# FengDushuo/BBBP-Multi-Modal-Deep-Ensemble-Framework

Hardware: AMD Instinct MI355X
Metric: molecules/sec fwd+bwd (3-branch ensemble, B=512) (higher is better)
Workload: dtype f32; 1 GPU; MixedInputModel F=167 (MACCS) + 3x128x128 image, 6-layer encoder + 2-stage CNN + fusion + BN head; forward + MSE + backward + fused AdamW, train mode (dropout 0.1); global_batch=512, per_gpu_batch=512, parallelism=dp1, input=device-resident

## Files before the change

### bbbp-multi-modal-deep-ensemble-framework_amd/csrc/head.hip

```cpp
#include "common.h"
#include "bbbp_hip.h"
#include "head_sync.h"

namespace {

constexpr int ROWS = 16;
constexpr int NTH = 512;
constexpr int NW = NTH / 64;
constexpr int COMB = 256, FHID = 128, NHEADS = 4, H1 = 256, H2 = 128, H3 = 64;
constexpr int LD = COMB + 4;
typedef float f32x4g __attribute__((ext_vector_type(4), aligned(4)));
static_assert(NTH >= H1, "one thread per BatchNorm column");

struct HeadParams {
    const float* comb;
    const float* fw1[NHEADS]; const float* fb1[NHEADS]; const float* fw2[NHEADS]; const float* fb2[NHEADS];
    const float* w0; const float* b0;
    const float* gamma; const float* beta; float* running_mean; float* running_var;
    const float* w3; const float* b3;
    const float* w5; const float* b5;
    const float* w7; const float* b7;
    float* hid; float* attn; float* fused; float* h; float* hb; float* bn_mean; float* bn_rstd; float* h2; float* h3; float* out;
    float* partial;
    int B, training;
    float eps, momentum;
    int concat;
    int world, rank;
};

template <int NCH>
__device__ __forceinline__ void load_b(f32x4 (&bf)[NCH], const float* Wrow ) {
#pragma unroll
    for (int c = 0; c < NCH; ++c) { f32x4g v = *reinterpret_cast<const f32x4g*>(Wrow + 16 * c); bf[c] = f32x4{v[0], v[1], v[2], v[3]}; }
}
template <int NCH>
__device__ __forceinline__ f32x4 mma_tile(const f32x4 (&af)[NCH], const f32x4 (&bf)[NCH]) {
    f32x4 acc0 = {0.f, 0.f, 0.f, 0.f}, acc1 = {0.f, 0.f, 0.f, 0.f};
#pragma unroll
    for (int c = 0; c < NCH; ++c)
#pragma unroll
        for (int j = 0; j < 4; j += 2) {
            acc0 = __builtin_amdgcn_mfma_f32_16x16x4f32(af[c][j], bf[c][j], acc0, 0, 0, 0);
            acc1 = __builtin_amdgcn_mfma_f32_16x16x4f32(af[c][j + 1], bf[c][j + 1], acc1, 0, 0, 0);
        }
    return acc0 + acc1;
}

template <int NCH>
__device__ __forceinline__ void load_a(f32x4 (&af)[NCH], const float* s, int ld, int lane) {
    const int i = lane & 15, kq = lane >> 4;
#pragma unroll
    for (int c = 0; c < NCH; ++c) af[c] = *reinterpret_cast<const f32x4*>(s + i * ld + 16 * c + 4 * kq);
}

__device__ __forceinline__ float sum16(float v) {
    v += __shfl_xor(v, 1); v += __shfl_xor(v, 2); v += __shfl_xor(v, 4); v += __shfl_xor(v, 8);
    return v;
}

__global__ __launch_bounds__(NTH) void head_a_kernel(HeadParams p) {
    __shared__ __attribute__((aligned(16))) float sC[ROWS * LD];
    __shared__ float sLogit[NW][NHEADS][ROWS];
    __shared__ float sP[ROWS][NHEADS];
    const int t = threadIdx.x, lane = t & 63, wave = t >> 6;
    const int q = lane & 15, kq = lane >> 4;
    const int r0 = blockIdx.x * ROWS, nrows = min(ROWS, p.B - r0);
    for (int idx = t; idx < ROWS * (COMB / 4); idx += NTH) {
        const int r = idx / (COMB / 4), c4 = idx % (COMB / 4);
        f32x4 v = {0.f, 0.f, 0.f, 0.f};
        if (r < nrows) v = *reinterpret_cast<const f32x4*>(p.comb + (long)(r0 + r) * COMB + c4 * 4);
        *reinterpret_cast<f32x4*>(sC + r * LD + c4 * 4) = v;
    }
    __syncthreads();
    f32x4 af[COMB / 16];
    load_a<COMB / 16>(af, sC, LD, lane);
    float lg[NHEADS][4];
    f32x4 bf[2][COMB / 16];
    const int n = wave * 16 + q;
    if (p.concat) {
        load_b<COMB / 16>(bf[0], p.w0 + (long)n * COMB + 4 * kq);
    } else {
    load_b<COMB / 16>(bf[0], p.fw1[0] + (long)n * COMB + 4 * kq);
#pragma unroll
    for (int h = 0; h < NHEADS; ++h) {
        if (h + 1 < NHEADS) load_b<COMB / 16>(bf[(h + 1) & 1], p.fw1[h + 1] + (long)n * COMB + 4 * kq);
        else load_b<COMB / 16>(bf[(h + 1) & 1], p.w0 + (long)n * COMB + 4 * kq);
        f32x4 acc = mma_tile<COMB / 16>(af, bf[h & 1]);
        const float b = p.fb1[h][n], w2 = p.fw2[h][n];
#pragma unroll
        for (int r = 0; r < 4; ++r) {
            const int row = 4 * kq + r;
            const float v = tanhf(acc[r] + b);
            if (row < nrows) p.hid[((long)h * p.B + r0 + row) * FHID + n] = v;
            lg[h][r] = sum16(v * w2);
        }
    }
    if (q == 0) {
#pragma unroll
        for (int h = 0; h < NHEADS; ++h)
#pragma unroll
            for (int r = 0; r < 4; ++r) sLogit[wave][h][4 * kq + r] = lg[h][r];
    }
    __syncthreads();
    if (t < ROWS) {
        float a[NHEADS], m = -INFINITY;
#pragma unroll
        for (int h = 0; h < NHEADS; ++h) {
            float z = 0.f;
#pragma unroll
            for (int w = 0; w < NW; ++w) z += sLogit[w][h][t];
            a[h] = z + p.fb2[h][0];
            m = fmaxf(m, a[h]);
        }
        float den = 0.f;
#pragma unroll
        for (int h = 0; h < NHEADS; ++h) { a[h] = __expf(a[h] - m); den += a[h]; }
#pragma unroll
        for (int h = 0; h < NHEADS; ++h) {
            a[h] /= den;
            sP[t][h] = a[h];
            if (t < nrows) p.attn[(long)(r0 + t) * NHEADS + h] = a[h];
        }
    }
    __syncthreads();
    for (int idx = t; idx < ROWS * COMB; idx += NTH) {
        const int r = idx / COMB, c = idx % COMB;
        const float x = sC[r * LD + c];
        float s = 0.f;
#pragma unroll
        for (int h = 0; h < NHEADS; ++h) s += sP[r][h] * x;
        sC[r * LD + c] = s;
        if (r < nrows) p.fused[(long)(r0 + r) * COMB + c] = s;
    }
    __syncthreads();
    load_a<COMB / 16>(af, sC, LD, lane);
    }
#pragma unroll
    for (int tt = 0; tt < 2; ++tt) {
        const int n0 = (wave + NW * tt) * 16 + q;
        if (tt == 0) load_b<COMB / 16>(bf[1], p.w0 + (long)((wave + NW) * 16 + q) * COMB + 4 * kq);
        f32x4 acc = mma_tile<COMB / 16>(af, bf[tt & 1]);
        const float b = p.b0[n0];
        float v[4], s = 0.f;
#pragma unroll
        for (int r = 0; r < 4; ++r) {
            const int row = 4 * kq + r;
            v[r] = fmaxf(acc[r] + b, 0.f);
            if (row < nrows) { p.h[(long)(r0 + row) * H1 + n0] = v[r]; s += v[r]; }
        }
        s += __shfl_xor(s, 16); s += __shfl_xor(s, 32);
        const float mean = s / nrows;
        float m2 = 0.f;
#pragma unroll
        for (int r = 0; r < 4; ++r) if (4 * kq + r < nrows) { const float d = v[r] - mean; m2 += d * d; }
        m2 += __shfl_xor(m2, 16); m2 += __shfl_xor(m2, 32);
        if (kq == 0) {
            const long slot = (long)p.rank * gridDim.x + blockIdx.x;
            p.partial[(slot * 2 + 0) * H1 + n0] = mean;
            p.partial[(slot * 2 + 1) * H1 + n0] = m2;
        }
    }
}

__global__ __launch_bounds__(NTH) void head_b_kernel(HeadParams p) {
    __shared__ __attribute__((aligned(16))) float sA[ROWS * LD];
    __shared__ __attribute__((aligned(16))) float sB[ROWS * (H2 + 4)];
    __shared__ __attribute__((aligned(16))) float sD[ROWS * (H3 + 4)];
    __shared__ float sMean[H1], sRstd[H1];
    const int t = threadIdx.x, lane = t & 63, wave = t >> 6;
    const int q = lane & 15, kq = lane >> 4;
    const int r0 = blockIdx.x * ROWS, nrows = min(ROWS, p.B - r0);
    const int nblocks = (p.B + ROWS - 1) / ROWS;
    f32x4 bf3[H1 / 16];
    load_b<H1 / 16>(bf3, p.w3 + (long)(wave * 16 + q) * H1 + 4 * kq);
    if (t < H1) {
        const int c = t;
        float mean, rstd;
        if (p.training) {
            float na = 0.f, ma = 0.f, m2a = 0.f;
            for (int b = 0; b < nblocks * p.world; ++b) {
                const float nb = (float)min(ROWS, p.B - (b % nblocks) * ROWS);
                const float mb = p.partial[((long)b * 2 + 0) * H1 + c], m2b = p.partial[((long)b * 2 + 1) * H1 + c];
                const float d = mb - ma, n = na + nb;
                ma += d * (nb / n);
                m2a += m2b + d * d * (na * nb / n);
                na = n;
            }
            const float nall = (float)p.B * (float)p.world;
            const float var = m2a / nall;
            mean = ma; rstd = rsqrtf(var + p.eps);
            if (blockIdx.x == 0) {
                p.running_mean[c] = (1.f - p.momentum) * p.running_mean[c] + p.momentum * mean;
                p.running_var[c] = (1.f - p.momentum) * p.running_var[c] + p.momentum * var * (nall / (nall - 1.f));
            }
        } else {
            mean = p.running_mean[c]; rstd = rsqrtf(p.running_var[c] + p.eps);
        }
        sMean[c] = mean; sRstd[c] = rstd;
        if (blockIdx.x == 0) { p.bn_mean[c] = mean; p.bn_rstd[c] = rstd; }
    }
    __syncthreads();
    for (int idx = t; idx < ROWS * H1; idx += NTH) {
        const int r = idx / H1, c = idx % H1;
        float v = 0.f;
        if (r < nrows) {
            v = (p.h[(long)(r0 + r) * H1 + c] - sMean[c]) * sRstd[c] * p.gamma[c] + p.beta[c];
            p.hb[(long)(r0 + r) * H1 + c] = v;
        }
        sA[r * LD + c] = v;
    }
    __syncthreads();
    {
        f32x4 af[H1 / 16];
        load_a<H1 / 16>(af, sA, LD, lane);
        const int n = wave * 16 + q;
        f32x4 acc = mma_tile<H1 / 16>(af, bf3);
        const float b = p.b3[n];
#pragma unroll
        for (int r = 0; r < 4; ++r) {
            const int row = 4 * kq + r;
            const float v = fmaxf(acc[r] + b, 0.f);
            sB[row * (H2 + 4) + n] = v;
            if (row < nrows) p.h2[(long)(r0 + row) * H2 + n] = v;
        }
    }
    __syncthreads();
    if (wave < H3 / 16) {
        f32x4 af[H2 / 16], bf[H2 / 16];
        const int n = wave * 16 + q;
        load_b<H2 / 16>(bf, p.w5 + (long)n * H2 + 4 * kq);
        load_a<H2 / 16>(af, sB, H2 + 4, lane);
        f32x4 acc = mma_tile<H2 / 16>(af, bf);
        const float b = p.b5[n];
#pragma unroll
        for (int r = 0; r < 4; ++r) {
            const int row = 4 * kq + r;
            const float v = fmaxf(acc[r] + b, 0.f);
            sD[row * (H3 + 4) + n] = v;
            if (row < nrows) p.h3[(long)(r0 + row) * H3 + n] = v;
        }
    }
    __syncthreads();
    if (wave == 0) {
        const int row = lane >> 2, part = lane & 3;
        float s = 0.f;
#pragma unroll
        for (int k = 0; k < H3 / 4; ++k) s += sD[row * (H3 + 4) + part * (H3 / 4) + k] * p.w7[part * (H3 / 4) + k];
        s += __shfl_xor(s, 1); s += __shfl_xor(s, 2);
        if (part == 0 && row < nrows) p.out[r0 + row] = s + p.b7[0];
    }
}

struct HeadBwdParams {
    const float* dout;
    const float* comb; const float* hid; const float* attn; const float* h; const float* h2; const float* h3;
    const float* bn_mean; const float* bn_rstd; const float* gamma;
    const float* fw1[NHEADS]; const float* fw2[NHEADS];
    const float* w0; const float* w3; const float* w5; const float* w7;
    float* dh3; float* dh2; float* dhb; float* dh; float* dlogit; float* dpre; float* dcomb;
    float* dgamma; float* dbeta;
    float* partial;
    int B, training;
    int world, rank;
};

typedef float f32x2g __attribute__((ext_vector_type(2), aligned(4)));

template <int K, int T>
__device__ __forceinline__ void mma_kmajor(f32x4 (&acc)[T], const float* sA, int lda, const float* W, int ldw, int colbase, int lane) {
    const int q = lane & 15, kq = lane >> 4;
    const float* wcol = W + colbase + T * q;
#pragma unroll 4
    for (int c = 0; c < K / 16; ++c) {
        const f32x4 a = *reinterpret_cast<const f32x4*>(sA + q * lda + 16 * c + 4 * kq);
#pragma unroll
        for (int j = 0; j < 4; ++j) {
            const float* wr = wcol + (long)(16 * c + 4 * kq + j) * ldw;
            if constexpr (T == 2) {
                const f32x2g b = *reinterpret_cast<const f32x2g*>(wr);
                acc[0] = __builtin_amdgcn_mfma_f32_16x16x4f32(a[j], b[0], acc[0], 0, 0, 0);
                acc[1] = __builtin_amdgcn_mfma_f32_16x16x4f32(a[j], b[1], acc[1], 0, 0, 0);
            } else {
                acc[0] = __builtin_amdgcn_mfma_f32_16x16x4f32(a[j], wr[0], acc[0], 0, 0, 0);
            }
        }
    }
}

constexpr int LD2 = H2 + 4, LD3 = H3 + 4, LDP = FHID + 4;

__global__ __launch_bounds__(NTH) void head_bwd_a_kernel(HeadBwdParams p) {
    __shared__ __attribute__((aligned(16))) float sD3[ROWS * LD3];
    __shared__ __attribute__((aligned(16))) float sD2[ROWS * LD2];
    __shared__ float sPa[4][H1], sPb[4][H1];
    const int t = threadIdx.x, lane = t & 63, wave = t >> 6;
    const int q = lane & 15, kq = lane >> 4;
    const int r0 = blockIdx.x * ROWS, nrows = min(ROWS, p.B - r0);
    for (int idx = t; idx < ROWS * H3; idx += NTH) {
        const int r = idx / H3, c = idx % H3;
        float v = 0.f;
        if (r < nrows) {
            v = p.h3[(long)(r0 + r) * H3 + c] > 0.f ? p.dout[r0 + r] * p.w7[c] : 0.f;
            p.dh3[(long)(r0 + r) * H3 + c] = v;
        }
        sD3[r * LD3 + c] = v;
    }
    __syncthreads();
    {
        f32x4 acc[1] = {{0.f, 0.f, 0.f, 0.f}};
        mma_kmajor<H3, 1>(acc, sD3, LD3, p.w5, H2, wave * 16, lane);
        const int n = wave * 16 + q;
#pragma unroll
        for (int r = 0; r < 4; ++r) {
            const int row = 4 * kq + r;
            float v = 0.f;
            if (row < nrows) {
                v = p.h2[(long)(r0 + row) * H2 + n] > 0.f ? acc[0][r] : 0.f;
                p.dh2[(long)(r0 + row) * H2 + n] = v;
            }
            sD2[row * LD2 + n] = v;
        }
    }
    __syncthreads();
    {
        f32x4 acc[2] = {{0.f, 0.f, 0.f, 0.f}, {0.f, 0.f, 0.f, 0.f}};
        mma_kmajor<H2, 2>(acc, sD2, LD2, p.w3, H1, wave * 32, lane);
#pragma unroll
        for (int u = 0; u < 2; ++u) {
            const int n = wave * 32 + 2 * q + u;
            const float mu = p.bn_mean[n], rs = p.bn_rstd[n];
            float pa = 0.f, pb = 0.f;
#pragma unroll
            for (int r = 0; r < 4; ++r) {
                const int row = 4 * kq + r;
                if (row < nrows) {
                    const float g = acc[u][r];
                    p.dhb[(long)(r0 + row) * H1 + n] = g;
                    pa += g * (p.h[(long)(r0 + row) * H1 + n] - mu) * rs;
                    pb += g;
                }
            }
            sPa[kq][n] = pa; sPb[kq][n] = pb;
        }
    }
    __syncthreads();
    if (t < H1) {
        const long slot = (long)p.rank * gridDim.x + blockIdx.x;
        p.partial[(slot * 2 + 0) * H1 + t] = ((sPa[0][t] + sPa[1][t]) + sPa[2][t]) + sPa[3][t];
        p.partial[(slot * 2 + 1) * H1 + t] = ((sPb[0][t] + sPb[1][t]) + sPb[2][t]) + sPb[3][t];
    }
}

__global__ __launch_bounds__(NTH) void head_bwd_c_kernel(HeadBwdParams p) {
    __shared__ __attribute__((aligned(16))) float sX[ROWS * LD];
    __shared__ __attribute__((aligned(16))) float sP[NHEADS * ROWS * LDP];
    __shared__ float sSa[H1], sSb[H1];
    const int t = threadIdx.x, lane = t & 63, wave = t >> 6;
    const int q = lane & 15, kq = lane >> 4;
    const int r0 = blockIdx.x * ROWS, nrows = min(ROWS, p.B - r0);
    const int nblocks = (p.B + ROWS - 1) / ROWS;
    if (t < H1) {
        float sa = 0.f, sb = 0.f, la = 0.f, lb = 0.f;
        for (int b = 0; b < nblocks * p.world; ++b) {
            const float va = p.partial[((long)b * 2 + 0) * H1 + t], vb = p.partial[((long)b * 2 + 1) * H1 + t];
            sa += va; sb += vb;
            if (b / nblocks == p.rank) { la += va; lb += vb; }
        }
        sSa[t] = sa; sSb[t] = sb;
        if (blockIdx.x == 0) { p.dgamma[t] = la; p.dbeta[t] = lb; }
    }
    __syncthreads();
    for (int idx = t; idx < ROWS * H1; idx += NTH) {
        const int r = idx / H1, c = idx % H1;
        float v = 0.f;
        if (r < nrows) {
            const float d = p.dhb[(long)(r0 + r) * H1 + c], xv = p.h[(long)(r0 + r) * H1 + c];
            const float g = p.gamma[c], mu = p.bn_mean[c], rs = p.bn_rstd[c];
            const float nall = (float)p.B * (float)p.world;
            v = p.training ? g * rs * (d - sSb[c] / nall - (xv - mu) * rs * (sSa[c] / nall)) : d * g * rs;
            v = xv > 0.f ? v : 0.f;
            p.dh[(long)(r0 + r) * H1 + c] = v;
        }
        sX[r * LD + c] = v;
    }
    __syncthreads();
    f32x4 df[2] = {{0.f, 0.f, 0.f, 0.f}, {0.f, 0.f, 0.f, 0.f}};
    mma_kmajor<H1, 2>(df, sX, LD, p.w0, COMB, wave * 32, lane);
    __syncthreads();
#pragma unroll
    for (int u = 0; u < 2; ++u)
#pragma unroll
        for (int r = 0; r < 4; ++r) sX[(4 * kq + r) * LD + wave * 32 + 2 * q + u] = df[u][r];
    __syncthreads();
#pragma unroll
    for (int rr = 0; rr < 2; ++rr) {
        const int r = wave * 2 + rr;
        const bool live = r < nrows;
        float a[NHEADS], asum = 0.f;
#pragma unroll
        for (int hh = 0; hh < NHEADS; ++hh) { a[hh] = live ? p.attn[(long)(r0 + r) * NHEADS + hh] : 0.f; asum += a[hh]; }
        float tt = 0.f;
#pragma unroll
        for (int c = lane; c < COMB; c += 64) {
            const float g = sX[r * LD + c];
            tt += live ? g * p.comb[(long)(r0 + r) * COMB + c] : 0.f;
            sX[r * LD + c] = g * asum;
        }
#pragma unroll
        for (int o = 32; o > 0; o >>= 1) tt += __shfl_xor(tt, o);
#pragma unroll
        for (int hh = 0; hh < NHEADS; ++hh) {
            const float dl = a[hh] * (tt - tt * asum);
            if (lane == 0 && live) p.dlogit[(long)hh * p.B + r0 + r] = dl;
#pragma unroll
            for (int c = lane; c < FHID; c += 64) {
                float v = 0.f;
                if (live) {
                    const float y = p.hid[((long)hh * p.B + r0 + r) * FHID + c];
                    v = dl * p.fw2[hh][c] * (1.f - y * y);
                    p.dpre[((long)hh * p.B + r0 + r) * FHID + c] = v;
                }
                sP[(hh * ROWS + r) * LDP + c] = v;
            }
        }
    }
    __syncthreads();
    f32x4 acc[2] = {{0.f, 0.f, 0.f, 0.f}, {0.f, 0.f, 0.f, 0.f}};
#pragma unroll
    for (int hh = 0; hh < NHEADS; ++hh) mma_kmajor<FHID, 2>(acc, sP + hh * ROWS * LDP, LDP, p.fw1[hh], COMB, wave * 32, lane);
#pragma unroll
    for (int u = 0; u < 2; ++u) {
        const int n = wave * 32 + 2 * q + u;
#pragma unroll
        for (int r = 0; r < 4; ++r) {
            const int row = 4 * kq + r;
            if (row < nrows) {
                const float v = acc[u][r] + sX[row * LD + n];
                p.dcomb[(long)(r0 + row) * COMB + n] = p.comb[(long)(r0 + row) * COMB + n] > 0.f ? v : 0.f;
            }
        }
    }
}

}

int bbbp_head_forward_fused(hipStream_t st, const float* comb, const float* const* fw1, const float* const* fb1,
                            const float* const* fw2, const float* const* fb2, const float* w0, const float* b0, const float* gamma,
                            const float* beta, float* running_mean, float* running_var, const float* w3, const float* b3,
                            const float* w5, const float* b5, const float* w7, const float* b7, float* hid, float* attn, float* fused,
                            float* h, float* hb, float* bn_mean, float* bn_rstd, float* h2, float* h3, float* out, float* partial,
                            int B, int training, int concat) {
    return bbbp_head_forward_fused_sync(st, comb, fw1, fb1, fw2, fb2, w0, b0, gamma, beta, running_mean, running_var, w3, b3, w5, b5, w7, b7,
                                        hid, attn, fused, h, hb, bn_mean, bn_rstd, h2, h3, out, partial, B, training, concat, nullptr);
}

int bbbp_head_forward_fused_sync(hipStream_t st, const float* comb, const float* const* fw1, const float* const* fb1,
                                 const float* const* fw2, const float* const* fb2, const float* w0, const float* b0, const float* gamma,
                                 const float* beta, float* running_mean, float* running_var, const float* w3, const float* b3,
                                 const float* w5, const float* b5, const float* w7, const float* b7, float* hid, float* attn, float* fused,
                                 float* h, float* hb, float* bn_mean, float* bn_rstd, float* h2, float* h3, float* out, float* partial,
                                 int B, int training, int concat, const bbbp_head_sync* sync) {
    const int world = sync ? sync->world : 1, rank = sync ? sync->rank : 0;
    BBBP_CHECK_ARG(B >= 1, "head: empty batch");
    BBBP_CHECK_ARG(world >= 1 && rank >= 0 && rank < world, "head: rank %d of %d", rank, world);
    BBBP_CHECK_ARG(!(training && (long)B * world <= 1), "Expected more than 1 value per channel when training, got input size [%d, %d]", B, H1);
    HeadParams p;
    p.comb = comb;
    for (int i = 0; i < NHEADS; ++i) { p.fw1[i] = fw1[i]; p.fb1[i] = fb1[i]; p.fw2[i] = fw2[i]; p.fb2[i] = fb2[i]; }
    p.w0 = w0; p.b0 = b0; p.gamma = gamma; p.beta = beta; p.running_mean = running_mean; p.running_var = running_var;
    p.w3 = w3; p.b3 = b3; p.w5 = w5; p.b5 = b5; p.w7 = w7; p.b7 = b7;
    p.hid = hid; p.attn = attn; p.fused = fused; p.h = h; p.hb = hb; p.bn_mean = bn_mean; p.bn_rstd = bn_rstd; p.h2 = h2; p.h3 = h3;
    p.out = out; p.partial = partial; p.B = B; p.training = training; p.eps = 1e-5f; p.momentum = 0.1f; p.concat = concat;
    p.world = world; p.rank = rank;
    const int blocks = cdiv(B, ROWS);
    hipLaunchKernelGGL(head_a_kernel, dim3(blocks), dim3(NTH), 0, st, p);
    BBBP_CHECK_LAUNCH();
    if (sync && sync->between && training) { const int rc = sync->between(); if (rc) return rc; }
    hipLaunchKernelGGL(head_b_kernel, dim3(blocks), dim3(NTH), 0, st, p);
    BBBP_CHECK_LAUNCH();
    return BBBP_OK;
}

int bbbp_head_backward_fused(hipStream_t st, const float* dout, const float* comb, const float* hid, const float* attn, const float* h,
                             const float* h2, const float* h3, const float* bn_mean, const float* bn_rstd, const float* gamma,
                             const float* const* fw1, const float* const* fw2, const float* w0, const float* w3, const float* w5,
                             const float* w7, float* dh3, float* dh2, float* dhb, float* dh, float* dlogit, float* dpre, float* dcomb,
                             float* dgamma, float* dbeta, float* partial, int B, int training) {
    return bbbp_head_backward_fused_sync(st, dout, comb, hid, attn, h, h2, h3, bn_mean, bn_rstd, gamma, fw1, fw2, w0, w3, w5, w7, dh3, dh2, dhb, dh,
                                         dlogit, dpre, dcomb, dgamma, dbeta, partial, B, training, nullptr);
}

int bbbp_head_backward_fused_sync(hipStream_t st, const float* dout, const float* comb, const float* hid, const float* attn, const float* h,
                                  const float* h2, const float* h3, const float* bn_mean, const float* bn_rstd, const float* gamma,
                                  const float* const* fw1, const float* const* fw2, const float* w0, const float* w3, const float* w5,
                                  const float* w7, float* dh3, float* dh2, float* dhb, float* dh, float* dlogit, float* dpre, float* dcomb,
                                  float* dgamma, float* dbeta, float* partial, int B, int training, const bbbp_head_sync* sync) {
    const int world = sync ? sync->world : 1, rank = sync ? sync->rank : 0;
    BBBP_CHECK_ARG(world >= 1 && rank >= 0 && rank < world, "head backward: rank %d of %d", rank, world);
    BBBP_CHECK_ARG(B >= 1, "head backward: empty batch");
    HeadBwdParams p;
    p.dout = dout; p.comb = comb; p.hid = hid; p.attn = attn; p.h = h; p.h2 = h2; p.h3 = h3;
    p.bn_mean = bn_mean; p.bn_rstd = bn_rstd; p.gamma = gamma;
    for (int i = 0; i < NHEADS; ++i) { p.fw1[i] = fw1[i]; p.fw2[i] = fw2[i]; }
    p.w0 = w0; p.w3 = w3; p.w5 = w5; p.w7 = w7;
    p.dh3 = dh3; p.dh2 = dh2; p.dhb = dhb; p.dh = dh; p.dlogit = dlogit; p.dpre = dpre; p.dcomb = dcomb;
    p.dgamma = dgamma; p.dbeta = dbeta; p.partial = partial; p.B = B; p.training = training;
    p.world = world; p.rank = rank;
    const int blocks = cdiv(B, ROWS);
    hipLaunchKernelGGL(head_bwd_a_kernel, dim3(blocks), dim3(NTH), 0, st, p);
    BBBP_CHECK_LAUNCH();
    if (sync && sync->between && training) { const int rc = sync->between(); if (rc) return rc; }
    hipLaunchKernelGGL(head_bwd_c_kernel, dim3(blocks), dim3(NTH), 0, st, p);
    BBBP_CHECK_LAUNCH();
    return BBBP_OK;
}

namespace {
bool four_pointers(const float* const* a) { return a && a[0] && a[1] && a[2] && a[3]; }
}

int bbbp_head_fwd(void* stream, const float* comb, const float* const* fw1, const float* const* fb1, const float* const* fw2,
                  const float* const* fb2, const float* w0, const float* b0, const float* gamma, const float* beta,
                  float* running_mean, float* running_var, const float* w3, const float* b3, const float* w5, const float* b5,
                  const float* w7, const float* b7, float* hid, float* attn, float* fused, float* h, float* hb, float* bn_mean,
                  float* bn_rstd, float* h2, float* h3, float* out, float* partial, int B, int training, int concat, int world, int rank) {
    BBBP_CHECK_ARG(comb && w0 && b0 && gamma && beta && running_mean && running_var && w3 && b3 && w5 && b5 && w7 && b7 && h && hb &&
                   bn_mean && bn_rstd && h2 && h3 && out && partial, "head_fwd: null pointer");
    BBBP_CHECK_ARG(concat || (four_pointers(fw1) && four_pointers(fb1) && four_pointers(fw2) && four_pointers(fb2) && hid && attn && fused),
                   "head_fwd: null pointer (the fusion block's parameters and outputs are required unless concat)");
    const float* const none[NHEADS] = {nullptr, nullptr, nullptr, nullptr};
    bbbp_head_sync sync;
    sync.world = world; sync.rank = rank;
    return bbbp_head_forward_fused_sync(static_cast<hipStream_t>(stream), comb, concat ? none : fw1, concat ? none : fb1, concat ? none : fw2,
                                        concat ? none : fb2, w0, b0, gamma, beta, running_mean, running_var, w3, b3, w5, b5, w7, b7, hid, attn,
                                        fused, h, hb, bn_mean, bn_rstd, h2, h3, out, partial, B, training, concat, &sync);
}

int bbbp_head_bwd(void* stream, const float* dout, const float* comb, const float* hid, const float* attn, const float* h,
                  const float* h2, const float* h3, const float* bn_mean, const float* bn_rstd, const float* gamma,
                  const float* const* fw1, const float* const* fw2, const float* w0, const float* w3, const float* w5,
                  const float* w7, float* dh3, float* dh2, float* dhb, float* dh, float* dlogit, float* dpre, float* dcomb,
                  float* dgamma, float* dbeta, float* partial, int B, int training, int world, int rank) {
    BBBP_CHECK_ARG(dout && comb && hid && attn && h && h2 && h3 && bn_mean && bn_rstd && gamma && four_pointers(fw1) && four_pointers(fw2) &&
                   w0 && w3 && w5 && w7 && dh3 && dh2 && dhb && dh && dlogit && dpre && dcomb && dgamma && dbeta && partial,
                   "head_bwd: null pointer");
    BBBP_CHECK_ARG(B >= 1, "head_bwd: empty batch");
    BBBP_CHECK_ARG(world >= 1 && rank >= 0 && rank < world, "head_bwd: rank %d of %d", rank, world);
    BBBP_CHECK_ARG(!(training && (long)B * world <= 1), "Expected more than 1 value per channel when training, got input size [%d, %d]", B, H1);
    bbbp_head_sync sync;
    sync.world = world; sync.rank = rank;
    return bbbp_head_backward_fused_sync(static_cast<hipStream_t>(stream), dout, comb, hid, attn, h, h2, h3, bn_mean, bn_rstd, gamma, fw1, fw2,
                                         w0, w3, w5, w7, dh3, dh2, dhb, dh, dlogit, dpre, dcomb, dgamma, dbeta, partial, B, training, &sync);
}
```

Before: 222,400 molecules/s.

## Prefetch head weights and activations into registers before barriers in head kernels

Across the head forward and backward kernels, global loads of weights, biases, activations and BN statistics are issued early into registers, ahead of __syncthreads and the reduction phases, so their latency overlaps other work. The Chan merge and partial-sum loops over per-block BN partials are batched in chunks of 32 loads before the dependent arithmetic. fw1 weight tiles are double-buffered across heads in the backward MFMA loop. Explicit contract-off helpers keep the float rounding order close to the original, at the cost of much higher register pressure and possibly lower occupancy.

```diff
diff --git a/bbbp-multi-modal-deep-ensemble-framework_amd/csrc/head.hip b/bbbp-multi-modal-deep-ensemble-framework_amd/csrc/head.hip
--- a/bbbp-multi-modal-deep-ensemble-framework_amd/csrc/head.hip
+++ b/bbbp-multi-modal-deep-ensemble-framework_amd/csrc/head.hip
@@ -10,7 +10,9 @@
 constexpr int COMB = 256, FHID = 128, NHEADS = 4, H1 = 256, H2 = 128, H3 = 64;
 constexpr int LD = COMB + 4;
 typedef float f32x4g __attribute__((ext_vector_type(4), aligned(4)));
+constexpr int MCH = 32;
 static_assert(NTH >= H1, "one thread per BatchNorm column");
+static_assert(NTH % H1 == 0, "row loops over [ROWS][H1]: a thread keeps its column in every trip");
 
 struct HeadParams {
     const float* comb;
@@ -58,6 +60,35 @@
     return v;
 }
 
+
+__device__ __forceinline__ void chan_merge(float& na, float& ma, float& m2a, float nb, float mb, float m2b, bool live) {
+#pragma clang fp contract(off)
+    const float d = mb - ma, n = na + nb;
+    const float ma1 = ma + d * (nb / n);
+    const float m2a1 = m2a + __builtin_fmaf(d * d, na * nb / n, m2b);
+    ma = live ? ma1 : ma; m2a = live ? m2a1 : m2a; na = live ? n : na;
+}
+__device__ __forceinline__ float bn_bwd_train(float d, float xv, float g, float mu, float rs, float qb, float qa) {
+#pragma clang fp contract(off)
+    return (g * rs) * ((d - qb) - ((xv - mu) * rs) * qa);
+}
+__device__ __forceinline__ float fusion_dot(const float (&g)[COMB / 64], const float (&c)[COMB / 64], bool live) {
+#pragma clang fp contract(off)
+    float tt = live ? __builtin_fmaf(g[0], c[0], 0.f) : 0.f;
+#pragma unroll
+    for (int k = 1; k < COMB / 64; ++k) tt = tt + (live ? g[k] * c[k] : 0.f);
+    return tt;
+}
+__device__ __forceinline__ float fusion_dlogit(float a, float tt, float asum) {
+#pragma clang fp contract(off)
+    return a * __builtin_fmaf(-asum, tt, tt);
+}
+__device__ __forceinline__ float fusion_dpre(float dl, float w2, float y, bool first) {
+#pragma clang fp contract(off)
+    const float s = first ? __builtin_fmaf(-y, y, 1.f) : 1.f - y * y;
+    return (dl * w2) * s;
+}
+
 __global__ __launch_bounds__(NTH) void head_a_kernel(HeadParams p) {
     __shared__ __attribute__((aligned(16))) float sC[ROWS * LD];
     __shared__ float sLogit[NW][NHEADS][ROWS];
@@ -65,28 +96,40 @@
     const int t = threadIdx.x, lane = t & 63, wave = t >> 6;
     const int q = lane & 15, kq = lane >> 4;
     const int r0 = blockIdx.x * ROWS, nrows = min(ROWS, p.B - r0);
-    for (int idx = t; idx < ROWS * (COMB / 4); idx += NTH) {
-        const int r = idx / (COMB / 4), c4 = idx % (COMB / 4);
-        f32x4 v = {0.f, 0.f, 0.f, 0.f};
-        if (r < nrows) v = *reinterpret_cast<const f32x4*>(p.comb + (long)(r0 + r) * COMB + c4 * 4);
-        *reinterpret_cast<f32x4*>(sC + r * LD + c4 * 4) = v;
+    constexpr int CTRIPS = ROWS * (COMB / 4) / NTH;
+    f32x4 cv[CTRIPS];
+#pragma unroll
+    for (int i = 0; i < CTRIPS; ++i) {
+        const int idx = t + i * NTH, r = idx / (COMB / 4), c4 = idx % (COMB / 4);
+        cv[i] = *reinterpret_cast<const f32x4*>(p.comb + (long)(r0 + min(r, nrows - 1)) * COMB + c4 * 4);
+    }
+    const int n = wave * 16 + q;
+    f32x4 bf[2][COMB / 16];
+    load_b<COMB / 16>(bf[0], (p.concat ? p.w0 : p.fw1[0]) + (long)n * COMB + 4 * kq);
+    float b0v[2], fb1v[NHEADS], fw2v[NHEADS], fb2v[NHEADS];
+#pragma unroll
+    for (int tt = 0; tt < 2; ++tt) b0v[tt] = p.b0[(wave + NW * tt) * 16 + q];
+    if (!p.concat) {
+#pragma unroll
+        for (int h = 0; h < NHEADS; ++h) { fb1v[h] = p.fb1[h][n]; fw2v[h] = p.fw2[h][n]; fb2v[h] = p.fb2[h][0]; }
+    }
+#pragma unroll
+    for (int i = 0; i < CTRIPS; ++i) {
+        const int idx = t + i * NTH, r = idx / (COMB / 4), c4 = idx % (COMB / 4);
+        const f32x4 zero = {0.f, 0.f, 0.f, 0.f};
+        *reinterpret_cast<f32x4*>(sC + r * LD + c4 * 4) = r < nrows ? cv[i] : zero;
     }
     __syncthreads();
     f32x4 af[COMB / 16];
     load_a<COMB / 16>(af, sC, LD, lane);
     float lg[NHEADS][4];
-    f32x4 bf[2][COMB / 16];
-    const int n = wave * 16 + q;
-    if (p.concat) {
-        load_b<COMB / 16>(bf[0], p.w0 + (long)n * COMB + 4 * kq);
-    } else {
-    load_b<COMB / 16>(bf[0], p.fw1[0] + (long)n * COMB + 4 * kq);
+    if (!p.concat) {
 #pragma unroll
     for (int h = 0; h < NHEADS; ++h) {
         if (h + 1 < NHEADS) load_b<COMB / 16>(bf[(h + 1) & 1], p.fw1[h + 1] + (long)n * COMB + 4 * kq);
         else load_b<COMB / 16>(bf[(h + 1) & 1], p.w0 + (long)n * COMB + 4 * kq);
         f32x4 acc = mma_tile<COMB / 16>(af, bf[h & 1]);
-        const float b = p.fb1[h][n], w2 = p.fw2[h][n];
+        const float b = fb1v[h], w2 = fw2v[h];
 #pragma unroll
         for (int r = 0; r < 4; ++r) {
             const int row = 4 * kq + r;
@@ -109,7 +152,7 @@
             float z = 0.f;
 #pragma unroll
             for (int w = 0; w < NW; ++w) z += sLogit[w][h][t];
-            a[h] = z + p.fb2[h][0];
+            a[h] = z + fb2v[h];
             m = fmaxf(m, a[h]);
         }
         float den = 0.f;
@@ -140,7 +183,7 @@
         const int n0 = (wave + NW * tt) * 16 + q;
         if (tt == 0) load_b<COMB / 16>(bf[1], p.w0 + (long)((wave + NW) * 16 + q) * COMB + 4 * kq);
         f32x4 acc = mma_tile<COMB / 16>(af, bf[tt & 1]);
-        const float b = p.b0[n0];
+        const float b = b0v[tt];
         float v[4], s = 0.f;
 #pragma unroll
         for (int r = 0; r < 4; ++r) {
@@ -173,18 +216,42 @@
     const int nblocks = (p.B + ROWS - 1) / ROWS;
     f32x4 bf3[H1 / 16];
     load_b<H1 / 16>(bf3, p.w3 + (long)(wave * 16 + q) * H1 + 4 * kq);
+    constexpr int TRIPS = ROWS * H1 / NTH, RSTEP = NTH / H1;
+    const int col = t % H1, rbase = t / H1;
+    float hv[TRIPS];
+#pragma unroll
+    for (int i = 0; i < TRIPS; ++i) hv[i] = p.h[(long)(r0 + min(rbase + RSTEP * i, nrows - 1)) * H1 + col];
+    const float gam = p.gamma[col], bet = p.beta[col];
+    const float b3v = p.b3[wave * 16 + q];
+    f32x4 bf5[H2 / 16];
+    load_b<H2 / 16>(bf5, p.w5 + (long)((wave % (H3 / 16)) * 16 + q) * H2 + 4 * kq);
+    const float b5v = p.b5[(wave % (H3 / 16)) * 16 + q];
+    float w7v[H3 / 4];
+#pragma unroll
+    for (int k = 0; k < H3 / 4; ++k) w7v[k] = p.w7[(lane & 3) * (H3 / 4) + k];
+    const float b7v = p.b7[0];
     if (t < H1) {
         const int c = t;
         float mean, rstd;
         if (p.training) {
+            const int total = nblocks * p.world;
+            const float ntail = (float)(p.B - (nblocks - 1) * ROWS);
             float na = 0.f, ma = 0.f, m2a = 0.f;
-            for (int b = 0; b < nblocks * p.world; ++b) {
-                const float nb = (float)min(ROWS, p.B - (b % nblocks) * ROWS);
-                const float mb = p.partial[((long)b * 2 + 0) * H1 + c], m2b = p.partial[((long)b * 2 + 1) * H1 + c];
-                const float d = mb - ma, n = na + nb;
-                ma += d * (nb / n);
-                m2a += m2b + d * d * (na * nb / n);
-                na = n;
+            for (int cb = 0; cb < total; cb += MCH) {
+                float mbv[MCH], m2bv[MCH];
+#pragma unroll
+                for (int i = 0; i < MCH; ++i) {
+                    const long b = min(cb + i, total - 1);
+                    mbv[i] = p.partial[(b * 2 + 0) * H1 + c]; m2bv[i] = p.partial[(b * 2 + 1) * H1 + c];
+                }
+                int bi = cb % nblocks;
+#pragma unroll
+                for (int i = 0; i < MCH; ++i) {
+                    const bool live = cb + i < total;
+                    const float nb = bi == nblocks - 1 ? ntail : (float)ROWS;
+                    bi = bi == nblocks - 1 ? 0 : bi + 1;
+                    chan_merge(na, ma, m2a, nb, mbv[i], m2bv[i], live);
+                }
             }
             const float nall = (float)p.B * (float)p.world;
             const float var = m2a / nall;
@@ -200,14 +267,15 @@
         if (blockIdx.x == 0) { p.bn_mean[c] = mean; p.bn_rstd[c] = rstd; }
     }
     __syncthreads();
-    for (int idx = t; idx < ROWS * H1; idx += NTH) {
-        const int r = idx / H1, c = idx % H1;
-        float v = 0.f;
-        if (r < nrows) {
-            v = (p.h[(long)(r0 + r) * H1 + c] - sMean[c]) * sRstd[c] * p.gamma[c] + p.beta[c];
-            p.hb[(long)(r0 + r) * H1 + c] = v;
-        }
-        sA[r * LD + c] = v;
+    {
+        const float mu = sMean[col], rs = sRstd[col];
+#pragma unroll
+        for (int i = 0; i < TRIPS; ++i) {
+            const int r = rbase + RSTEP * i;
+            const float v = r < nrows ? (hv[i] - mu) * rs * gam + bet : 0.f;
+            if (r < nrows) p.hb[(long)(r0 + r) * H1 + col] = v;
+            sA[r * LD + col] = v;
+        }
     }
     __syncthreads();
     {
@@ -215,7 +283,7 @@
         load_a<H1 / 16>(af, sA, LD, lane);
         const int n = wave * 16 + q;
         f32x4 acc = mma_tile<H1 / 16>(af, bf3);
-        const float b = p.b3[n];
+        const float b = b3v;
 #pragma unroll
         for (int r = 0; r < 4; ++r) {
             const int row = 4 * kq + r;
@@ -226,12 +294,11 @@
     }
     __syncthreads();
     if (wave < H3 / 16) {
-        f32x4 af[H2 / 16], bf[H2 / 16];
+        f32x4 af[H2 / 16];
         const int n = wave * 16 + q;
-        load_b<H2 / 16>(bf, p.w5 + (long)n * H2 + 4 * kq);
         load_a<H2 / 16>(af, sB, H2 + 4, lane);
-        f32x4 acc = mma_tile<H2 / 16>(af, bf);
-        const float b = p.b5[n];
+        f32x4 acc = mma_tile<H2 / 16>(af, bf5);
+        const float b = b5v;
 #pragma unroll
         for (int r = 0; r < 4; ++r) {
             const int row = 4 * kq + r;
@@ -245,9 +312,9 @@
         const int row = lane >> 2, part = lane & 3;
         float s = 0.f;
 #pragma unroll
-        for (int k = 0; k < H3 / 4; ++k) s += sD[row * (H3 + 4) + part * (H3 / 4) + k] * p.w7[part * (H3 / 4) + k];
+        for (int k = 0; k < H3 / 4; ++k) s += sD[row * (H3 + 4) + part * (H3 / 4) + k] * w7v[k];
         s += __shfl_xor(s, 1); s += __shfl_xor(s, 2);
-        if (part == 0 && row < nrows) p.out[r0 + row] = s + p.b7[0];
+        if (part == 0 && row < nrows) p.out[r0 + row] = s + b7v;
     }
 }
 
@@ -267,23 +334,32 @@
 typedef float f32x2g __attribute__((ext_vector_type(2), aligned(4)));
 
 template <int K, int T>
-__device__ __forceinline__ void mma_kmajor(f32x4 (&acc)[T], const float* sA, int lda, const float* W, int ldw, int colbase, int lane) {
+__device__ __forceinline__ void load_kmajor(float (&w)[K / 4][T], const float* W, int ldw, int colbase, int lane) {
     const int q = lane & 15, kq = lane >> 4;
     const float* wcol = W + colbase + T * q;
-#pragma unroll 4
-    for (int c = 0; c < K / 16; ++c) {
-        const f32x4 a = *reinterpret_cast<const f32x4*>(sA + q * lda + 16 * c + 4 * kq);
+#pragma unroll
+    for (int c = 0; c < K / 16; ++c)
 #pragma unroll
         for (int j = 0; j < 4; ++j) {
             const float* wr = wcol + (long)(16 * c + 4 * kq + j) * ldw;
             if constexpr (T == 2) {
                 const f32x2g b = *reinterpret_cast<const f32x2g*>(wr);
-                acc[0] = __builtin_amdgcn_mfma_f32_16x16x4f32(a[j], b[0], acc[0], 0, 0, 0);
-                acc[1] = __builtin_amdgcn_mfma_f32_16x16x4f32(a[j], b[1], acc[1], 0, 0, 0);
+                w[4 * c + j][0] = b[0]; w[4 * c + j][1] = b[1];
             } else {
-                acc[0] = __builtin_amdgcn_mfma_f32_16x16x4f32(a[j], wr[0], acc[0], 0, 0, 0);
-            }
-        }
+                w[4 * c + j][0] = wr[0];
+            }
+        }
+}
+template <int K, int T>
+__device__ __forceinline__ void mma_kmajor(f32x4 (&acc)[T], const float* sA, int lda, const float (&w)[K / 4][T], int lane) {
+    const int q = lane & 15, kq = lane >> 4;
+#pragma unroll
+    for (int c = 0; c < K / 16; ++c) {
+        const f32x4 a = *reinterpret_cast<const f32x4*>(sA + q * lda + 16 * c + 4 * kq);
+#pragma unroll
+        for (int j = 0; j < 4; ++j)
+#pragma unroll
+            for (int u = 0; u < T; ++u) acc[u] = __builtin_amdgcn_mfma_f32_16x16x4f32(a[j], w[4 * c + j][u], acc[u], 0, 0, 0);
     }
 }
 
@@ -296,39 +372,56 @@
     const int t = threadIdx.x, lane = t & 63, wave = t >> 6;
     const int q = lane & 15, kq = lane >> 4;
     const int r0 = blockIdx.x * ROWS, nrows = min(ROWS, p.B - r0);
-    for (int idx = t; idx < ROWS * H3; idx += NTH) {
-        const int r = idx / H3, c = idx % H3;
-        float v = 0.f;
-        if (r < nrows) {
-            v = p.h3[(long)(r0 + r) * H3 + c] > 0.f ? p.dout[r0 + r] * p.w7[c] : 0.f;
-            p.dh3[(long)(r0 + r) * H3 + c] = v;
-        }
-        sD3[r * LD3 + c] = v;
+    constexpr int TRIPS = ROWS * H3 / NTH, RSTEP = NTH / H3;
+    const int col = t % H3, rbase = t / H3;
+    float h3v[TRIPS], doutv[TRIPS];
+#pragma unroll
+    for (int i = 0; i < TRIPS; ++i) {
+        const int rc = r0 + min(rbase + RSTEP * i, nrows - 1);
+        h3v[i] = p.h3[(long)rc * H3 + col]; doutv[i] = p.dout[rc];
+    }
+    const float w7c = p.w7[col];
+    float w5r[H3 / 4][1], w3r[H2 / 4][2];
+    load_kmajor<H3, 1>(w5r, p.w5, H2, wave * 16, lane);
+    load_kmajor<H2, 2>(w3r, p.w3, H1, wave * 32, lane);
+    float h2v[4], hv[2][4], muv[2], rsv[2];
+#pragma unroll
+    for (int r = 0; r < 4; ++r) {
+        const long rc = r0 + min(4 * kq + r, nrows - 1);
+        h2v[r] = p.h2[rc * H2 + wave * 16 + q];
+#pragma unroll
+        for (int u = 0; u < 2; ++u) hv[u][r] = p.h[rc * H1 + wave * 32 + 2 * q + u];
+    }
+#pragma unroll
+    for (int u = 0; u < 2; ++u) { muv[u] = p.bn_mean[wave * 32 + 2 * q + u]; rsv[u] = p.bn_rstd[wave * 32 + 2 * q + u]; }
+#pragma unroll
+    for (int i = 0; i < TRIPS; ++i) {
+        const int r = rbase + RSTEP * i;
+        const float v = r < nrows ? (h3v[i] > 0.f ? doutv[i] * w7c : 0.f) : 0.f;
+        if (r < nrows) p.dh3[(long)(r0 + r) * H3 + col] = v;
+        sD3[r * LD3 + col] = v;
     }
     __syncthreads();
     {
         f32x4 acc[1] = {{0.f, 0.f, 0.f, 0.f}};
-        mma_kmajor<H3, 1>(acc, sD3, LD3, p.w5, H2, wave * 16, lane);
+        mma_kmajor<H3, 1>(acc, sD3, LD3, w5r, lane);
         const int n = wave * 16 + q;
 #pragma unroll
         for (int r = 0; r < 4; ++r) {
             const int row = 4 * kq + r;
-            float v = 0.f;
-            if (row < nrows) {
-                v = p.h2[(long)(r0 + row) * H2 + n] > 0.f ? acc[0][r] : 0.f;
-                p.dh2[(long)(r0 + row) * H2 + n] = v;
-            }
+            const float v = row < nrows ? (h2v[r] > 0.f ? acc[0][r] : 0.f) : 0.f;
+            if (row < nrows) p.dh2[(long)(r0 + row) * H2 + n] = v;
             sD2[row * LD2 + n] = v;
         }
     }
     __syncthreads();
     {
         f32x4 acc[2] = {{0.f, 0.f, 0.f, 0.f}, {0.f, 0.f, 0.f, 0.f}};
-        mma_kmajor<H2, 2>(acc, sD2, LD2, p.w3, H1, wave * 32, lane);
+        mma_kmajor<H2, 2>(acc, sD2, LD2, w3r, lane);
 #pragma unroll
         for (int u = 0; u < 2; ++u) {
             const int n = wave * 32 + 2 * q + u;
-            const float mu = p.bn_mean[n], rs = p.bn_rstd[n];
+            const float mu = muv[u], rs = rsv[u];
             float pa = 0.f, pb = 0.f;
 #pragma unroll
             for (int r = 0; r < 4; ++r) {
@@ -336,7 +429,7 @@
                 if (row < nrows) {
                     const float g = acc[u][r];
                     p.dhb[(long)(r0 + row) * H1 + n] = g;
-                    pa += g * (p.h[(long)(r0 + row) * H1 + n] - mu) * rs;
+                    pa += g * (hv[u][r] - mu) * rs;
                     pb += g;
                 }
             }
@@ -359,33 +452,76 @@
     const int q = lane & 15, kq = lane >> 4;
     const int r0 = blockIdx.x * ROWS, nrows = min(ROWS, p.B - r0);
     const int nblocks = (p.B + ROWS - 1) / ROWS;
+    float w0r[H1 / 4][2];
+    load_kmajor<H1, 2>(w0r, p.w0, COMB, wave * 32, lane);
+    constexpr int TRIPS = ROWS * H1 / NTH, RSTEP = NTH / H1;
+    const int col = t % H1, rbase = t / H1;
+    float dv[TRIPS], xvv[TRIPS];
+#pragma unroll
+    for (int i = 0; i < TRIPS; ++i) {
+        const long rc = r0 + min(rbase + RSTEP * i, nrows - 1);
+        dv[i] = p.dhb[rc * H1 + col]; xvv[i] = p.h[rc * H1 + col];
+    }
+    const float g = p.gamma[col], mu = p.bn_mean[col], rs = p.bn_rstd[col];
     if (t < H1) {
+        const int total = nblocks * p.world, mine = p.rank * nblocks;
         float sa = 0.f, sb = 0.f, la = 0.f, lb = 0.f;
-        for (int b = 0; b < nblocks * p.world; ++b) {
-            const float va = p.partial[((long)b * 2 + 0) * H1 + t], vb = p.partial[((long)b * 2 + 1) * H1 + t];
-            sa += va; sb += vb;
-            if (b / nblocks == p.rank) { la += va; lb += vb; }
+        for (int cb = 0; cb < total; cb += MCH) {
+            float vav[MCH], vbv[MCH];
+#pragma unroll
+            for (int i = 0; i < MCH; ++i) {
+                const long b = min(cb + i, total - 1);
+                vav[i] = p.partial[(b * 2 + 0) * H1 + t]; vbv[i] = p.partial[(b * 2 + 1) * H1 + t];
+            }
+#pragma unroll
+            for (int i = 0; i < MCH; ++i) {
+                const int b = cb + i;
+                const bool live = b < total, local = live && b >= mine && b < mine + nblocks;
+                const float va = vav[i], vb = vbv[i];
+                sa = live ? sa + va : sa; sb = live ? sb + vb : sb;
+                la = local ? la + va : la; lb = local ? lb + vb : lb;
+            }
         }
         sSa[t] = sa; sSb[t] = sb;
         if (blockIdx.x == 0) { p.dgamma[t] = la; p.dbeta[t] = lb; }
     }
     __syncthreads();
-    for (int idx = t; idx < ROWS * H1; idx += NTH) {
-        const int r = idx / H1, c = idx % H1;
-        float v = 0.f;
-        if (r < nrows) {
-            const float d = p.dhb[(long)(r0 + r) * H1 + c], xv = p.h[(long)(r0 + r) * H1 + c];
-            const float g = p.gamma[c], mu = p.bn_mean[c], rs = p.bn_rstd[c];
-            const float nall = (float)p.B * (float)p.world;
-            v = p.training ? g * rs * (d - sSb[c] / nall - (xv - mu) * rs * (sSa[c] / nall)) : d * g * rs;
+    {
+        const float nall = (float)p.B * (float)p.world;
+        const float ssa = sSa[col], ssb = sSb[col];
+#pragma unroll
+        for (int i = 0; i < TRIPS; ++i) {
+            const int r = rbase + RSTEP * i;
+            const float d = dv[i], xv = xvv[i];
+            float v = p.training ? bn_bwd_train(d, xv, g, mu, rs, ssb / nall, ssa / nall) : d * g * rs;
             v = xv > 0.f ? v : 0.f;
-            p.dh[(long)(r0 + r) * H1 + c] = v;
-        }
-        sX[r * LD + c] = v;
-    }
+            v = r < nrows ? v : 0.f;
+            if (r < nrows) p.dh[(long)(r0 + r) * H1 + col] = v;
+            sX[r * LD + col] = v;
+        }
+    }
+    float at[2][NHEADS], cmb[2][COMB / 64], hidv[2][NHEADS][FHID / 64], fw2v[NHEADS][FHID / 64];
+#pragma unroll
+    for (int rr = 0; rr < 2; ++rr) {
+        const long rc = r0 + min(wave * 2 + rr, nrows - 1);
+#pragma unroll
+        for (int hh = 0; hh < NHEADS; ++hh) {
+            at[rr][hh] = p.attn[rc * NHEADS + hh];
+#pragma unroll
+            for (int k = 0; k < FHID / 64; ++k) hidv[rr][hh][k] = p.hid[((long)hh * p.B + rc) * FHID + lane + 64 * k];
+        }
+#pragma unroll
+        for (int k = 0; k < COMB / 64; ++k) cmb[rr][k] = p.comb[rc * COMB + lane + 64 * k];
+    }
+#pragma unroll
+    for (int hh = 0; hh < NHEADS; ++hh)
+#pragma unroll
+        for (int k = 0; k < FHID / 64; ++k) fw2v[hh][k] = p.fw2[hh][lane + 64 * k];
     __syncthreads();
     f32x4 df[2] = {{0.f, 0.f, 0.f, 0.f}, {0.f, 0.f, 0.f, 0.f}};
-    mma_kmajor<H1, 2>(df, sX, LD, p.w0, COMB, wave * 32, lane);
+    mma_kmajor<H1, 2>(df, sX, LD, w0r, lane);
+    float w1r[2][FHID / 4][2];
+    load_kmajor<FHID, 2>(w1r[0], p.fw1[0], COMB, wave * 32, lane);
     __syncthreads();
 #pragma unroll
     for (int u = 0; u < 2; ++u)
@@ -398,36 +534,42 @@
         const bool live = r < nrows;
         float a[NHEADS], asum = 0.f;
 #pragma unroll
-        for (int hh = 0; hh < NHEADS; ++hh) { a[hh] = live ? p.attn[(long)(r0 + r) * NHEADS + hh] : 0.f; asum += a[hh]; }
-        float tt = 0.f;
-#pragma unroll
-        for (int c = lane; c < COMB; c += 64) {
-            const float g = sX[r * LD + c];
-            tt += live ? g * p.comb[(long)(r0 + r) * COMB + c] : 0.f;
-            sX[r * LD + c] = g * asum;
-        }
+        for (int hh = 0; hh < NHEADS; ++hh) { a[hh] = live ? at[rr][hh] : 0.f; asum += a[hh]; }
+        float gx[COMB / 64];
+#pragma unroll
+        for (int k = 0; k < COMB / 64; ++k) {
+            gx[k] = sX[r * LD + lane + 64 * k];
+            sX[r * LD + lane + 64 * k] = gx[k] * asum;
+        }
+        float tt = fusion_dot(gx, cmb[rr], live);
 #pragma unroll
         for (int o = 32; o > 0; o >>= 1) tt += __shfl_xor(tt, o);
 #pragma unroll
         for (int hh = 0; hh < NHEADS; ++hh) {
-            const float dl = a[hh] * (tt - tt * asum);
+            const float dl = fusion_dlogit(a[hh], tt, asum);
             if (lane == 0 && live) p.dlogit[(long)hh * p.B + r0 + r] = dl;
 #pragma unroll
-            for (int c = lane; c < FHID; c += 64) {
-                float v = 0.f;
-                if (live) {
-                    const float y = p.hid[((long)hh * p.B + r0 + r) * FHID + c];
-                    v = dl * p.fw2[hh][c] * (1.f - y * y);
-                    p.dpre[((long)hh * p.B + r0 + r) * FHID + c] = v;
-                }
+            for (int k = 0; k < FHID / 64; ++k) {
+                const int c = lane + 64 * k;
+                const float v = live ? fusion_dpre(dl, fw2v[hh][k], hidv[rr][hh][k], k == 0) : 0.f;
+                if (live) p.dpre[((long)hh * p.B + r0 + r) * FHID + c] = v;
                 sP[(hh * ROWS + r) * LDP + c] = v;
             }
         }
     }
+    float cm[2][4];
+#pragma unroll
+    for (int r = 0; r < 4; ++r)
+#pragma unroll
+        for (int u = 0; u < 2; ++u) cm[u][r] = p.comb[(long)(r0 + min(4 * kq + r, nrows - 1)) * COMB + wave * 32 + 2 * q + u];
     __syncthreads();
     f32x4 acc[2] = {{0.f, 0.f, 0.f, 0.f}, {0.f, 0.f, 0.f, 0.f}};
 #pragma unroll
-    for (int hh = 0; hh < NHEADS; ++hh) mma_kmajor<FHID, 2>(acc, sP + hh * ROWS * LDP, LDP, p.fw1[hh], COMB, wave * 32, lane);
+    for (int hh = 0; hh < NHEADS; ++hh) {
+        if (hh + 1 < NHEADS) load_kmajor<FHID, 2>(w1r[(hh + 1) & 1], p.fw1[hh + 1], COMB, wave * 32, lane);
+        __builtin_amdgcn_sched_barrier(0);
+        mma_kmajor<FHID, 2>(acc, sP + hh * ROWS * LDP, LDP, w1r[hh & 1], lane);
+    }
 #pragma unroll
     for (int u = 0; u < 2; ++u) {
         const int n = wave * 32 + 2 * q + u;
@@ -436,7 +578,7 @@
             const int row = 4 * kq + r;
             if (row < nrows) {
                 const float v = acc[u][r] + sX[row * LD + n];
-                p.dcomb[(long)(r0 + row) * COMB + n] = p.comb[(long)(r0 + row) * COMB + n] > 0.f ? v : 0.f;
+                p.dcomb[(long)(r0 + row) * COMB + n] = cm[u][r] > 0.f ? v : 0.f;
             }
         }
     }
```

Result: no change. 224,700 molecules/s, median of 6 (+1.0%).
